# xxxupeng/stereo_toolbox

Hardware: AMD Instinct MI355X
Metric: stereo pairs/sec @ 540x960 D=192 (GwcNet_GC fwd+bwd) (higher is better)
Workload: dtype f32; 1 GPU; GwcNet_GC(maxdisp=192) train step: fwd+bwd+allreduce+Adam, 576x960 pairs (reference pad_to_2x shape), batch 1/GPU, fp32, synthetic randn inputs, deterministic filler weights; global_batch=1, parallelism=dp1, grad_sync=none (single rank: flat fp32 buffer packed, no collective), launch=eager, optimizer=torch.optim.Adam(fused=True)

## Files before the change

### include/stx_hip.h

```cpp
#ifndef STX_HIP_H
#define STX_HIP_H
#ifdef __cplusplus
extern "C" {
#endif

const char* stx_last_error(void);
const char* stx_build_info(void);
int stx_get_tuning(const char* name);
int stx_set_tuning(const char* name, int value);

int stx_cost_volume_fwd(const float* Lg, const float* Rg, int Cg, int G, const float* Lc, const float* Rc, int Cc,
                        const float* scale, float* vol, int B, int H, int W, int D, int mask_left, void* stream);
int stx_group_normalize_fwd(const float* x, float* y, int B, int C, int G, int HW, float out_scale, void* stream);
int stx_group_normalize_bwd(const float* x, const float* gy, float* gx, int B, int C, int G, int HW, float out_scale, void* stream);
int stx_cost_volume_bwd(const float* gvol, const float* Lg, const float* Rg, int Cg, int G, int Cc, float* gLg,
                        float* gRg, float* gLc, float* gRc, int B, int H, int W, int D, int mask_left, void* stream);

int stx_head_fwd(const float* cost, float* disp, float* stats, int B, int Dc, int Hc, int Wc, int D, int H, int W,
                 void* stream);
long long stx_head_bwd_workspace_floats(int B, int Dc, int H, int W);
int stx_head_bwd(const float* gdisp, const float* cost, const float* disp, const float* stats, float* gcost,
                 float* workspace, int B, int Dc, int Hc, int Wc, int D, int H, int W, void* stream);
int stx_head_fwd2(const float* cost, float* disp, float* stats, int B, int Dc, int Hc, int Wc, int D, int H, int W,
                  int align_corners, void* stream);
// ... 9 lines not shown
int stx_softmax_d_fwd(const float* x, float* y, int B, int D, int HW, void* stream);

long long stx_conv3d_packed_floats(int K, int N, int T);
int stx_conv3d_pack_weight(const float* w, float* wp, int A, int B, int T, int mode, void* stream);
int stx_conv3d_fwd_blocks(int Do, int Ho, int Wo);
long long stx_conv3d_fwd_stat_rows(int B, int Di, int Hi, int Wi, int Cin, int Cout, int ks, int stride);
int stx_conv3d_fwd(const float* x, const float* wp, float* out, const float* scale, const float* bias,
                   const float* residual, float* stats, int B, int Di, int Hi, int Wi, int Cin, int Cout, int ks,
                   int stride, int relu, void* stream);
int stx_deconv3d_fwd_blocks(int Di, int Hi, int Wi);
int stx_deconv3d_fwd(const float* x, const float* wp, float* out, const float* scale, const float* bias,
                     const float* residual, float* stats, int B, int Di, int Hi, int Wi, int Cin, int Cout, int Do,
                     int Ho, int Wo, int relu, void* stream);
long long stx_conv3d_wgrad_workspace_floats(int B, int Dc, int Hc, int Wc, int CF, int CC, int ks, int stride);
int stx_conv3d_wgrad(const float* fine, const float* coarse, float* dw, float* workspace, int B, int Df, int Hf, int Wf,
                     int CF, int Dc, int Hc, int Wc, int CC, int ks, int stride, void* stream);

int stx_conv3d_wgrad_bn_supported(int B, int D, int H, int W, int CF, int CC);
int stx_conv3d_wgrad_bn(const float* x, const float* gy, const float* z, const float* scale, const float* shift, const float* mean,
                        const float* invstd, const float* gamma, const float* sums, float inv_n, int act, float* dz, float* dw,
                        float* workspace, int B, int D, int H, int W, int CF, int CC, void* stream);

int stx_conv2d_supported(int Cin, int Cout);
long long stx_conv2d_stat_rows(int groups);
int stx_conv2d_fwd(const float* x, const float* w, float* out, float* stats, int B, int H, int W, int Cin, int Cout, int dgrad,
                   int groups, void* stream);

int stx_conv3d_c1_fwd(const float* x, const float* w, const float* residual, float* out, int B, int D, int H, int W,
                      int Cin, void* stream);
long long stx_conv3d_c1_wgrad_workspace_floats(int Cin);
int stx_conv3d_c1_wgrad(const float* x, const float* gy, float* dw, float* workspace, int B, int D, int H, int W,
                        int Cin, void* stream);
int stx_conv3d_c1_dgrad(const float* gy, const float* w, float* gx, int B, int D, int H, int W, int Cin, void* stream);

int stx_mish_fwd(const float* x, float* y, long long n, void* stream);
int stx_mish_bwd(const float* gy, const float* x, float* gx, long long n, void* stream);
int stx_depth_to_space(const float* y, float* out, int B, int D, int H, int W, int C, int inverse, void* stream);
int stx_gate_fwd(const float* cv, const float* att, float* out, int B, int D, long long HW, int C, void* stream);
int stx_gate_bwd(const float* g, const float* cv, const float* att, float* gcv, float* gatt, int B, int D, long long HW,
                 int C, void* stream);

int stx_concat_channels(const float* in0, const float* in1, const float* in2, const float* in3, int C0, int C1, int C2, int C3,
                        float* out, long long nvox, void* stream);
int stx_split_channels(const float* in, float* out0, float* out1, float* out2, float* out3, int C0, int C1, int C2, int C3,
                       long long nvox, void* stream);
int stx_transpose(const float* in, float* out, int N, int rows, int cols, void* stream);

int stx_dwconv_hw_fwd(const float* x, const float* w, const int* dil, float* out, int B, int D, int H, int W, int C,
                      int flip, void* stream);
long long stx_dwconv_hw_wgrad_workspace_floats(int C);
int stx_dwconv_hw_wgrad(const float* x, const float* gy, const int* dil, float* dw, float* workspace, int B, int D,
                        int H, int W, int C, void* stream);
int stx_cost_volume_scale_bwd(const float* gvol, const float* Lc, const float* Rc, float* gscale, int B, int Cc, int H,
                              int W, int D, int mask_left, void* stream);
int stx_scale_channels(const float* x, const float* s, float* out, long long nvox, int C, void* stream);
int stx_ac_volume_bwd(const float* gvol, const float* Lc, const float* Rc, const float* prob, float* gL, float* gR,
                      float* gprob, int B, int Cc, int H, int W, int D, int mask_left, void* stream);

int stx_bn_reduce_blocks(void);
int stx_bn_stats_rows(long long nvox, int C);
int stx_bn_stats(const float* z, float* partials, long long nvox, int C, int groups, void* stream);
int stx_bn_finalize(const float* partials, int nrows, int C, double count, const float* gamma, const float* beta,
                    float* running_mean, float* running_var, float momentum, float eps, float* scale, float* shift,
                    float* mean, float* invstd, void* stream);
int stx_bn_finalize_groups(const float* partials, int nrows, int C, double count, const float* gamma, const float* beta,
                           float* running_mean, float* running_var, float momentum, float eps, float* out, int groups,
// ... 102 lines not shown
```

### stereo_toolbox_amd/_capi.py

```python
import ctypes
import os
import threading

import torch

_P = ctypes.c_void_p
_I = ctypes.c_int
_F = ctypes.c_float
_L = ctypes.c_longlong

SIGNATURES = {
    "stx_get_tuning": [ctypes.c_char_p],
    "stx_set_tuning": [ctypes.c_char_p, _I],
    "stx_cost_volume_fwd": [_P, _P, _I, _I, _P, _P, _I, _P, _P, _I, _I, _I, _I, _I, _P],
    "stx_cost_volume_bwd": [_P, _P, _P, _I, _I, _I, _P, _P, _P, _P, _I, _I, _I, _I, _I, _P],
    "stx_group_normalize_fwd": [_P, _P, _I, _I, _I, _I, _F, _P],
    "stx_group_normalize_bwd": [_P, _P, _P, _I, _I, _I, _I, _F, _P],
    "stx_head_fwd": [_P, _P, _P, _I, _I, _I, _I, _I, _I, _I, _P],
    "stx_head_bwd_workspace_floats": [_I, _I, _I, _I],
    "stx_head_bwd": [_P, _P, _P, _P, _P, _P, _I, _I, _I, _I, _I, _I, _I, _P],
    "stx_head_fwd2": [_P, _P, _P, _I, _I, _I, _I, _I, _I, _I, _I, _P],
    "stx_head_bwd2": [_P, _P, _P, _P, _P, _P, _I, _I, _I, _I, _I, _I, _I, _I, _P],
    "stx_softargmax_fwd": [_P, _P, _I, _I, _I, _P],
    "stx_argmax_fwd": [_P, _P, _I, _I, _I, _P],
    "stx_softmax_d_fwd": [_P, _P, _I, _I, _I, _P],
    "stx_unimodal_fwd": [_P, _P, _I, _I, _I, _P],
    "stx_dominant_modal_fwd": [_P, _P, _I, _I, _I, _P],
    "stx_modal_fwd": [_P, _P, _P, _I, _I, _I, _I, _P],
    "stx_modal_bwd": [_P, _P, _P, _P, _I, _I, _I, _P],
    "stx_split_mode": [_P, _P, _P, _I, _I, _I, _P],
    "stx_conv3d_packed_floats": [_I, _I, _I],
    "stx_conv3d_pack_weight": [_P, _P, _I, _I, _I, _I, _P],
    "stx_conv3d_fwd_blocks": [_I, _I, _I],
    "stx_conv3d_fwd_stat_rows": [_I, _I, _I, _I, _I, _I, _I, _I],
    "stx_deconv3d_fwd_blocks": [_I, _I, _I],
    "stx_conv3d_fwd": [_P, _P, _P, _P, _P, _P, _P, _I, _I, _I, _I, _I, _I, _I, _I, _I, _P],
    "stx_deconv3d_fwd": [_P, _P, _P, _P, _P, _P, _P, _I, _I, _I, _I, _I, _I, _I, _I, _I, _I, _P],
    "stx_conv3d_wgrad_workspace_floats": [_I, _I, _I, _I, _I, _I, _I, _I],
    "stx_conv3d_wgrad": [_P, _P, _P, _P, _I, _I, _I, _I, _I, _I, _I, _I, _I, _I, _I, _P],
    "stx_conv3d_wgrad_bn_supported": [_I, _I, _I, _I, _I, _I],
    "stx_conv3d_wgrad_bn": [_P] * 9 + [_F, _I, _P, _P, _P, _I, _I, _I, _I, _I, _I, _P],
    "stx_conv2d_supported": [_I, _I],
    "stx_conv2d_stat_rows": [_I],
    "stx_conv2d_fwd": [_P, _P, _P, _P, _I, _I, _I, _I, _I, _I, _I, _P],
    "stx_conv3d_c1_fwd": [_P, _P, _P, _P, _I, _I, _I, _I, _I, _P],
    "stx_conv3d_c1_wgrad_workspace_floats": [_I],
    "stx_conv3d_c1_wgrad": [_P, _P, _P, _P, _I, _I, _I, _I, _I, _P],
    "stx_conv3d_c1_dgrad": [_P, _P, _P, _I, _I, _I, _I, _I, _P],
    "stx_mish_fwd": [_P, _P, _L, _P],
    "stx_mish_bwd": [_P, _P, _P, _L, _P],
    "stx_depth_to_space": [_P, _P, _I, _I, _I, _I, _I, _I, _P],
    "stx_gate_fwd": [_P, _P, _P, _I, _I, _L, _I, _P],
    "stx_gate_bwd": [_P, _P, _P, _P, _P, _I, _I, _L, _I, _P],
    "stx_concat_channels": [_P, _P, _P, _P, _I, _I, _I, _I, _P, _L, _P],
    "stx_split_channels": [_P, _P, _P, _P, _P, _I, _I, _I, _I, _L, _P],
    "stx_transpose": [_P, _P, _I, _I, _I, _P],
    "stx_dwconv_hw_fwd": [_P, _P, _P, _P, _I, _I, _I, _I, _I, _I, _P],
    "stx_dwconv_hw_wgrad_workspace_floats": [_I],
    "stx_dwconv_hw_wgrad": [_P, _P, _P, _P, _P, _I, _I, _I, _I, _I, _P],
    "stx_cost_volume_scale_bwd": [_P, _P, _P, _P, _I, _I, _I, _I, _I, _I, _P],
    "stx_scale_channels": [_P, _P, _P, _L, _I, _P],
    "stx_ac_volume_bwd": [_P, _P, _P, _P, _P, _P, _P, _I, _I, _I, _I, _I, _I, _P],
    "stx_pad_normalize_u8": [_P, _P, _I, _I, _I, _I, _I, _I, _P, _P, _P],
    "stx_warp_fwd": [_P, _P, _P, _I, _I, _I, _I, _P],
    "stx_warp_bwd": [_P, _P, _P, _P, _P, _I, _I, _I, _I, _P],
    "stx_corr_volume_fwd": [_P, _P, _P, _I, _I, _I, _I, _I, _I, _P],
    "stx_corr_volume_bwd": [_P, _P, _P, _P, _P, _I, _I, _I, _I, _I, _I, _P],
    "stx_disparity_variance_fwd": [_P, _P, _P, _P, _I, _I, _I, _P],
    "stx_disparity_variance_bwd": [_P, _P, _P, _P, _P, _P, _P, _I, _I, _I, _P],
    "stx_sampled_volume_fwd": [_P, _P, _I, _I, _P, _P, _I, _P, _P, _I, _I, _I, _I, _I, _P],
    "stx_sampled_volume_bwd": [_P, _P, _P, _I, _I, _I, _P, _P, _P, _P, _P, _I, _I, _I, _I, _I, _P],
    "stx_geo_pyramid_floats": [_L, _I, _I, _I],
    "stx_geo_corr_fwd": [_P, _P, _P, _I, _I, _I, _I, _I, _I, _P],
    "stx_geo_corr_bwd": [_P, _P, _P, _P, _P, _I, _I, _I, _I, _I, _I, _P],
    "stx_geo_pyramid_fwd": [_P, _P, _I, _I, _I, _I, _I, _I, _P],
    "stx_geo_pyramid_bwd": [_P, _P, _I, _I, _I, _I, _I, _I, _P],
    "stx_geo_lookup_fwd": [_P, _P, _P, _P, _P, _I, _I, _I, _I, _I, _I, _I, _I, _P],
    "stx_geo_lookup_bwd": [_P, _P, _P, _P, _P, _I, _I, _I, _I, _I, _I, _I, _I, _P],
    "stx_context_upsample_fwd": [_P, _P, _P, _I, _I, _I, _P],
    "stx_context_upsample_bwd": [_P, _P, _P, _P, _P, _I, _I, _I, _P],
    "stx_corr1d_pyramid_floats": [_L, _I, _I],
# ... 101 lines not shown
```

### stereo_toolbox_amd/aggregation.py

```python
import os
import threading

import torch
import torch.nn as nn

from . import ops


def _is_transposed(conv):
    return isinstance(conv, nn.ConvTranspose3d)


def _conv_cfg(conv):
    ks = conv.kernel_size[0]
    stride = conv.stride[0]
    if _is_transposed(conv):
        k3 = ks == 3 and stride == 2 and conv.padding[0] == 1 and conv.output_padding[0] == 1
        k4 = ks == 4 and stride == 2 and conv.padding[0] == 1 and conv.output_padding[0] == 0
        if not (k3 or k4) or len(set(conv.kernel_size)) != 1 or len(set(conv.stride)) != 1:
            raise ops.StxError("only ConvTranspose3d(k=3, s=2, p=1, op=1) and ConvTranspose3d(k=4, s=2, p=1) are on the hot path")
    else:
        if not ((ks == 3 and conv.padding[0] == 1 and stride in (1, 2)) or (ks == 1 and conv.padding[0] == 0 and stride == 1)):
            raise ops.StxError(f"unsupported Conv3d k={ks} s={stride} p={conv.padding}")
    if conv.bias is not None or conv.groups != 1:
# ... 160 lines not shown
        return _infer_conv(x, conv, s1, b1, residual, relu)

    want = bn is not None and bn.training
    z1, part1 = raw if raw is not None else _raw_conv(x, conv, want)
    if bn is None:
        y = z1
        if residual is not None:
            y = y + residual
        if relu == 3:
            return torch.nn.functional.leaky_relu(y, 0.01)
        return torch.relu(y) if relu else y
    count1 = z1.numel() // z1.shape[-1]
    st1 = _bn_state(bn, part1 if want else None, count1)
    if second is not None:
        x2, conv2, bn2 = second
        want2 = bn2.training
        z2, part2 = second_raw if second_raw is not None else _raw_conv(x2, conv2, want2)
        st2 = _bn_state(bn2, part2 if want2 else None, z2.numel() // z2.shape[-1])
        return ops.BnActFn.apply(z1, bn.weight, bn.bias, z2, bn2.weight, bn2.bias, None, relu, st1, st2)
    defer = (residual is None and want and relu in (0, 1, False, True) and not _is_transposed(conv) and _conv_cfg(conv) == (3, 1)
             and conv.weight.shape[0] % 32 == 0 and conv.weight.shape[1] % 32 == 0 and not st1.get("sync")
             and os.environ.get("STX_BN_BWD_IN_WGRAD", "1") != "0")
    if defer:
        ops.bn_defer_reset_if_stale()
    return ops.BnActFn.apply(z1, bn.weight, bn.bias, None, None, None, residual, relu, st1, None, 1, defer)


@ops.fp32_region
def convbn_block(x, seq, relu=False, second=None, residual=None, mish=False, raw=None, second_raw=None):
    sec = None
    if second is not None:
        sec = (second[0], second[1][0], second[1][1])
    return conv_block(x, seq[0], seq[1], relu=relu, second=sec, residual=residual, mish=mish, raw=raw, second_raw=second_raw)
```

### stereo_toolbox_amd/csrc/conv_c1.hip

```cpp
#include "stx_common.h"
#include <stdlib.h>

namespace {

constexpr int C1_THREADS = 256;
constexpr int C1_TD = 2, C1_TH = 4, C1_TW = 32;
constexpr int C1_ED = C1_TD + 2, C1_EH = C1_TH + 2, C1_EW = C1_TW + 2;
constexpr int C1_CK = 16, C1_VS = C1_CK + 4;

struct C1Args {
    const float* x;
    const float* w;
    const float* gy;
    const float* res;
    float* out;
    int B, D, H, W, Cin;
    int nDt, nHt, nWt, ntiles;
};

__device__ __forceinline__ void c1_stage(const C1Args& a, float* tile, int b, int d0, int h0, int w0, int c0, int tid) {
    for (int idx = tid; idx < C1_ED * C1_EH * C1_EW * (C1_CK / 4); idx += C1_THREADS) {
        const int v = idx / (C1_CK / 4), f = idx - v * (C1_CK / 4);
        const int wx = v % C1_EW, hy = (v / C1_EW) % C1_EH, dz = v / (C1_EW * C1_EH);
        const int gd = d0 - 1 + dz, gh = h0 - 1 + hy, gw = w0 - 1 + wx;
// ... 286 lines not shown
            for (int p = 0; p < 16; ++p) {
                float bv = gp[2 * p];
                bv = (i < 27) ? bv : 0.f;
                acc = __builtin_amdgcn_mfma_f32_32x32x2f32(av[p], bv, acc, 0, 0, 0);
            }
        }
    }
#pragma unroll
    for (int r = 0; r < 16; ++r) red[wave][((r & 3) + 8 * (r >> 2) + 4 * half) * 32 + i] = acc[r];
    __syncthreads();
    float* dst = slab + ((size_t)cb * gridDim.x + blockIdx.x) * 1024;
    for (int idx = tid; idx < 1024; idx += C1_THREADS)
        dst[idx] = (red[0][idx] + red[1][idx]) + (red[2][idx] + red[3][idx]);
}

__global__ __launch_bounds__(C1_THREADS) void c1m_reduce_kernel(const float* __restrict__ slab, int nrows,
                                                                float* __restrict__ dw) {
    __shared__ double red[C1_THREADS];
    const int m = blockIdx.x, tid = threadIdx.x;
    const int tap = m % 27, cfull = m / 27, cb = cfull >> 5, c = cfull & 31;
    const float* p = slab + (size_t)cb * nrows * 1024 + c * 32 + tap;
    double s = 0.0;
    for (int r = tid; r < nrows; r += C1_THREADS) s += (double)p[(size_t)r * 1024];
    red[tid] = s;
    __syncthreads();
    for (int k = C1_THREADS / 2; k > 0; k >>= 1) {
        if (tid < k) red[tid] += red[tid + k];
        __syncthreads();
    }
    if (tid == 0) dw[m] = (float)red[0];
}


constexpr int C1F_TH = 8, C1F_TW = 32;
constexpr int C1F_EH = C1F_TH + 2, C1F_EW = C1F_TW + 2, C1F_NV = C1F_EH * C1F_EW;
constexpr int C1F_MT = (C1F_NV + 31) / 32;
constexpr int C1F_WGS = 512;

__global__ __launch_bounds__(C1_THREADS) void conv_c1_fwd_mfma_kernel(const float* __restrict__ x,
                                                                      const float* __restrict__ w,
                                                                      const float* __restrict__ res,
                                                                      float* __restrict__ out, int B, int D, int H, int W,
                                                                      int nHt, int nWt, int ncols) {
    STX_DYN_SMEM(smem);
    float* Ps = reinterpret_cast<float*>(smem);
    const int tid = threadIdx.x, lane = tid & 63, wave = __builtin_amdgcn_readfirstlane(tid >> 6);
    const int i = lane & 31, half = lane >> 5;
    float wreg[16];
#pragma unroll
    for (int s_ = 0; s_ < 16; ++s_) wreg[s_] = (i < 27) ? w[(size_t)(16 * half + s_) * 27 + i] : 0.f;
    const int lh = tid / C1F_TW, lw = tid % C1F_TW;

    constexpr int MTW = (C1F_MT + 3) / 4;
    const long long units = (long long)ncols * D;
    int u = __builtin_amdgcn_readfirstlane((int)(units * blockIdx.x / gridDim.x));
    const int u_end = __builtin_amdgcn_readfirstlane((int)(units * (blockIdx.x + 1) / gridDim.x));
    const unsigned plane_bytes = (unsigned)H * (unsigned)W * 32u * 4u;
    while (u < u_end) {
        const int col = u / D;
        const int d_lo = u - col * D;
        const int left = u_end - u;
        const int d_hi = (D - d_lo < left) ? D : d_lo + left;
        u += d_hi - d_lo;
        const int wt = col % nWt, ht = (col / nWt) % nHt, b = col / (nWt * nHt);
        const int h0 = ht * C1F_TH, w0 = wt * C1F_TW;
        const int oh = h0 + lh, ow = w0 + lw;
        const bool ook = oh < H && ow < W;
        unsigned voff[MTW];
#pragma unroll
        for (int t = 0; t < MTW; ++t) {
            const int hv = (wave + 4 * t) * 32 + i;
            const int hy = hv / C1F_EW, wx = hv - hy * C1F_EW;
            const int gh = h0 - 1 + hy, gw = w0 - 1 + wx;
            const bool ok = wave + 4 * t < C1F_MT && hv < C1F_NV && gh >= 0 && gh < H && gw >= 0 && gw < W;
            voff[t] = ok ? (unsigned)(((gh * W + gw) * 32 + 16 * half) * 4) : STX_BUF_OOB;
        }
        float4 nxt[MTW][4];
        auto load_plane = [&](int p) {
            const bool in = p >= 0 && p < D && p <= d_hi;
            const stx_bufrsrc rs = stx_make_rsrc(x + ((size_t)b * D + (in ? p : 0)) * H * W * 32, in ? plane_bytes : 0u);
#pragma unroll
            for (int t = 0; t < MTW; ++t)
#pragma unroll
                for (int q = 0; q < 4; ++q) nxt[t][q] = stx_buf_ld4(rs, voff[t], 16u * q);
        };
        float accA = 0.f, accB = 0.f;
        load_plane(d_lo - 1);
        __syncthreads();
        for (int p = d_lo - 1; p <= d_hi; ++p) {
            float* Pb = Ps + ((p + 2) & 1) * (C1F_NV * 27);
            const bool pin = p >= 0 && p < D;
            float4 cur[MTW][4];
#pragma unroll
            for (int t = 0; t < MTW; ++t)
#pragma unroll
                for (int q = 0; q < 4; ++q) cur[t][q] = nxt[t][q];
            load_plane(p + 1);
            if (pin) {
#pragma unroll
                for (int t = 0; t < MTW; ++t) {
                    const int m = wave + 4 * t;
                    if (m < C1F_MT) {
                        f32x16 acc;
#pragma unroll
                        for (int r = 0; r < 16; ++r) acc[r] = 0.f;
#pragma unroll
                        for (int q = 0; q < 4; ++q) {
                            acc = __builtin_amdgcn_mfma_f32_32x32x2f32(cur[t][q].x, wreg[4 * q + 0], acc, 0, 0, 0);
                            acc = __builtin_amdgcn_mfma_f32_32x32x2f32(cur[t][q].y, wreg[4 * q + 1], acc, 0, 0, 0);
                            acc = __builtin_amdgcn_mfma_f32_32x32x2f32(cur[t][q].z, wreg[4 * q + 2], acc, 0, 0, 0);
                            acc = __builtin_amdgcn_mfma_f32_32x32x2f32(cur[t][q].w, wreg[4 * q + 3], acc, 0, 0, 0);
                        }
                        if (i < 27) {
#pragma unroll
                            for (int r = 0; r < 16; ++r) {
                                const int v = m * 32 + (r & 3) + 8 * (r >> 2) + 4 * half;
                                if (v < C1F_NV) Pb[v * 27 + i] = acc[r];
                            }
                        }
                    }
                }
            }
            __syncthreads();
            float s0 = 0.f, s1 = 0.f, s2 = 0.f;
            if (pin) {
#pragma unroll
                for (int kh = 0; kh < 3; ++kh)
#pragma unroll
                    for (int kw = 0; kw < 3; ++kw) {
                        const float* pp = Pb + ((lh + kh) * C1F_EW + lw + kw) * 27 + kh * 3 + kw;
                        s0 += pp[0];
                        s1 += pp[9];
                        s2 += pp[18];
                    }
            }
            const float done = accA + s2;
            const int od = p - 1;
            if (od >= d_lo && od < d_hi && ook) {
                const size_t o = (((size_t)b * D + od) * H + oh) * W + ow;
                out[o] = res ? done + res[o] : done;
            }
            accA = accB + s1;
            accB = s0;
        }
    }
}

}

extern "C" int stx_conv3d_c1_fwd(const float* x, const float* w, const float* residual, float* out, int B, int D,
                                 int H, int W, int Cin, void* stream) {
    stx_begin();
    STX_REQUIRE(x && w && out && B > 0 && D > 0 && H > 0 && W > 0, "conv3d_c1_fwd: bad shape");
    STX_REQUIRE(Cin % C1_CK == 0, "conv3d_c1_fwd: Cin=%d must be a multiple of %d", Cin, C1_CK);
    if (Cin == 32 && (long long)H * W * 128 < (1ll << 31)) {
        const int nHt = stx_cdiv(H, C1F_TH), nWt = stx_cdiv(W, C1F_TW);
        const long long ncols = (long long)B * nHt * nWt, units = ncols * D;
        STX_REQUIRE(units < (1ll << 31), "conv3d_c1_fwd: volume too large");
        long long g = C1F_WGS;
        if (g > units / 4) g = units / 4 > 0 ? units / 4 : 1;
        const size_t lds = (size_t)2 * C1F_NV * 27 * 4;
        if (int rc = stx_lds_require((const void*)conv_c1_fwd_mfma_kernel, lds, "conv3d_c1_fwd(mfma)")) return rc;
        hipLaunchKernelGGL(conv_c1_fwd_mfma_kernel, dim3((unsigned)g), dim3(C1_THREADS), lds, (hipStream_t)stream, x, w,
                           residual, out, B, D, H, W, nHt, nWt, (int)ncols);
        return stx_check_launch("conv3d_c1_fwd(mfma)");
    }
    C1Args a;
    a.x = x; a.w = w; a.gy = nullptr; a.res = residual; a.out = out;
    a.B = B; a.D = D; a.H = H; a.W = W; a.Cin = Cin;
    a.nDt = stx_cdiv(D, C1_TD); a.nHt = stx_cdiv(H, C1_TH); a.nWt = stx_cdiv(W, C1_TW);
    a.ntiles = B * a.nDt * a.nHt * a.nWt;
    if (int rc = stx_lds_require((const void*)conv_c1_fwd_kernel, C1_TILE_BYTES, "conv3d_c1_fwd")) return rc;
    hipLaunchKernelGGL(conv_c1_fwd_kernel, dim3(a.ntiles), dim3(C1_THREADS), C1_TILE_BYTES, (hipStream_t)stream, a);
    return stx_check_launch("conv3d_c1_fwd");
}

extern "C" long long stx_conv3d_c1_wgrad_workspace_floats(int Cin) {
    const long long valu = (long long)C1_WGRAD_BLOCKS * Cin * 27;
    const long long mfma = (long long)C1M_BLOCKS * 1024 * ((Cin + 31) / 32);
    return valu > mfma ? valu : mfma;
}

extern "C" int stx_conv3d_c1_wgrad(const float* x, const float* gy, float* dw, float* workspace, int B, int D, int H,
                                   int W, int Cin, void* stream) {
    stx_begin();
    STX_REQUIRE(x && gy && dw && workspace && B > 0, "conv3d_c1_wgrad: null operand");
    STX_REQUIRE(Cin % C1_CK == 0 && Cin <= 4 * C1_CK, "conv3d_c1_wgrad: Cin=%d must be 16..64 in steps of 16", Cin);
    if (Cin % 32 == 0) {
        const int nDt = stx_cdiv(D, C1M_TD), nHt = stx_cdiv(H, C1M_TH), nWt = stx_cdiv(W, C1M_TW);
        const long long nt = (long long)B * nDt * nHt * nWt;
        STX_REQUIRE(nt < (1ll << 31), "conv3d_c1_wgrad: volume too large");
        const int nblk = nt < C1M_BLOCKS ? (int)nt : C1M_BLOCKS;
        hipStream_t st = (hipStream_t)stream;
        hipLaunchKernelGGL(conv_c1_wgrad_mfma_kernel, dim3(nblk, Cin / 32), dim3(C1_THREADS), 0, st, x, gy, workspace, B,
                           D, H, W, Cin, nDt, nHt, nWt, (int)nt);
        int rc = stx_check_launch("conv3d_c1_wgrad(mfma)");
        if (rc) return rc;
        hipLaunchKernelGGL(c1m_reduce_kernel, dim3(Cin * 27), dim3(C1_THREADS), 0, st, workspace, nblk, dw);
        return stx_check_launch("conv3d_c1_wgrad(reduce)");
    }
    C1Args a;
    a.x = x; a.w = nullptr; a.gy = gy; a.res = nullptr; a.out = workspace;
    a.B = B; a.D = D; a.H = H; a.W = W; a.Cin = Cin;
    a.nDt = stx_cdiv(D, C1_TD); a.nHt = stx_cdiv(H, C1_TH); a.nWt = stx_cdiv(W, C1_TW);
    a.ntiles = B * a.nDt * a.nHt * a.nWt;
    const int nblk = a.ntiles < C1_WGRAD_BLOCKS ? a.ntiles : C1_WGRAD_BLOCKS;
    const size_t lds = C1_TILE_BYTES + 256 * 4;
// ... 26 lines not shown
```

### stereo_toolbox_amd/models/GwcNet/gwcnet.py

```python
import torch
import torch.nn as nn

from ... import ops
from ...aggregation import conv_block, convbn_block, deferred_bn_counters, shared_input_convs
from ..features2d import ResTrunk, cat_features, channels_last_weights_, convbn, init_reference_style, run_head2d, run_pair
from .submodule import convbn_3d


class feature_extraction(ResTrunk):
    fused_everywhere = True

    def __init__(self, concat_feature=False, concat_feature_channel=12):
        super().__init__()
        self.concat_feature = concat_feature
        if concat_feature:
            self.lastconv = nn.Sequential(convbn(320, 128, 3, 1, 1, 1), nn.ReLU(inplace=True),
                                          nn.Conv2d(128, concat_feature_channel, 1, bias=False))

    def forward(self, x):
        gwc = cat_features(self.trunk(x))
        if not self.concat_feature:
            return {"gwc_feature": gwc}
        return {"gwc_feature": gwc, "concat_feature": run_head2d(self.lastconv, gwc)}


class hourglass(nn.Module):

    def __init__(self, c):
        super().__init__()
        self.conv1 = nn.Sequential(convbn_3d(c, c * 2, 3, 2, 1), nn.ReLU(inplace=True))
        self.conv2 = nn.Sequential(convbn_3d(c * 2, c * 2, 3, 1, 1), nn.ReLU(inplace=True))
        self.conv3 = nn.Sequential(convbn_3d(c * 2, c * 4, 3, 2, 1), nn.ReLU(inplace=True))
        self.conv4 = nn.Sequential(convbn_3d(c * 4, c * 4, 3, 1, 1), nn.ReLU(inplace=True))
        self.conv5 = nn.Sequential(nn.ConvTranspose3d(c * 4, c * 2, 3, padding=1, output_padding=1, stride=2, bias=False),
                                   nn.BatchNorm3d(c * 2))
        self.conv6 = nn.Sequential(nn.ConvTranspose3d(c * 2, c, 3, padding=1, output_padding=1, stride=2, bias=False),
                                   nn.BatchNorm3d(c))
        self.redir1 = convbn_3d(c, c, kernel_size=1, stride=1, pad=0)
        self.redir2 = convbn_3d(c * 2, c * 2, kernel_size=1, stride=1, pad=0)

    def forward(self, x, mid=None, also=None):
        rx = shared_input_convs(x, [self.conv1[0], self.redir1] + ([also] if also is not None else []))
        rx = rx or [None, None, None]
        c1 = convbn_block(x, self.conv1[0], relu=True, raw=rx[0])
        c2 = convbn_block(c1, self.conv2[0], relu=True)
        r2 = shared_input_convs(c2, [self.conv3[0], self.redir2]) or [None, None]
        c3 = convbn_block(c2, self.conv3[0], relu=True, raw=r2[0])
        c4 = convbn_block(c3, self.conv4[0], relu=True)
        if mid is not None:
            c4 = mid(c4)
        c5 = convbn_block(c4, self.conv5, relu=True, second=(c2, self.redir2), second_raw=r2[1])
        out = convbn_block(c5, self.conv6, relu=True, second=(x, self.redir1), second_raw=rx[1])
        return (out, rx[2]) if also is not None else out


def classifier(c):
    return nn.Sequential(convbn_3d(c, c, 3, 1, 1), nn.ReLU(inplace=True),
                         nn.Conv3d(c, 1, kernel_size=3, padding=1, stride=1, bias=False))


def run_classifier(seq, x, add=None, raw=None):
    h = convbn_block(x, seq[0], relu=True, raw=raw)
    cost = conv_block(h, seq[2], residual=None if add is None else add.unsqueeze(-1))
    return cost.squeeze(-1)


class GwcNet(nn.Module):
    def __init__(self, maxdisp, use_concat_volume=False):
        super().__init__()
        self.maxdisp = maxdisp
        self.use_concat_volume = use_concat_volume
        self.num_groups = 40
        if use_concat_volume:
            self.concat_channels = 12
            self.feature_extraction = feature_extraction(True, self.concat_channels)
        else:
            self.concat_channels = 0
            self.feature_extraction = feature_extraction(False)
        self.dres0 = nn.Sequential(convbn_3d(self.num_groups + self.concat_channels * 2, 32, 3, 1, 1),
                                   nn.ReLU(inplace=True), convbn_3d(32, 32, 3, 1, 1), nn.ReLU(inplace=True))
        self.dres1 = nn.Sequential(convbn_3d(32, 32, 3, 1, 1), nn.ReLU(inplace=True), convbn_3d(32, 32, 3, 1, 1))
        self.dres2 = hourglass(32)
        self.dres3 = hourglass(32)
        self.dres4 = hourglass(32)
        self.classif0 = classifier(32)
        self.classif1 = classifier(32)
        self.classif2 = classifier(32)
        self.classif3 = classifier(32)
        init_reference_style(self)
        channels_last_weights_(self.feature_extraction)

    def forward(self, left, right):
        with deferred_bn_counters():
            fl, fr = run_pair(self.feature_extraction, left, right, self.training)
            return self.aggregate(fl, fr, left.shape[2], left.shape[3])

# ... 28 lines not shown
```

### stereo_toolbox_amd/models/PSMNet/stackhourglass.py

```python
import torch.nn as nn

from ... import ops
from ...aggregation import conv_block, convbn_block, deferred_bn_counters
from ..features2d import channels_last_weights_, init_reference_style, run_pair
from .submodule import convbn_3d, feature_extraction


class hourglass(nn.Module):

    def __init__(self, inplanes):
        super().__init__()
        c = inplanes
        self.conv1 = nn.Sequential(convbn_3d(c, c * 2, kernel_size=3, stride=2, pad=1), nn.ReLU(inplace=True))
        self.conv2 = convbn_3d(c * 2, c * 2, kernel_size=3, stride=1, pad=1)
        self.conv3 = nn.Sequential(convbn_3d(c * 2, c * 2, kernel_size=3, stride=2, pad=1), nn.ReLU(inplace=True))
        self.conv4 = nn.Sequential(convbn_3d(c * 2, c * 2, kernel_size=3, stride=1, pad=1), nn.ReLU(inplace=True))
        self.conv5 = nn.Sequential(nn.ConvTranspose3d(c * 2, c * 2, kernel_size=3, padding=1, output_padding=1,
                                                      stride=2, bias=False), nn.BatchNorm3d(c * 2))
        self.conv6 = nn.Sequential(nn.ConvTranspose3d(c * 2, c, kernel_size=3, padding=1, output_padding=1,
                                                      stride=2, bias=False), nn.BatchNorm3d(c))

    def forward(self, x, presqu, postsqu, skip=None):
        out = convbn_block(x, self.conv1[0], relu=True)
        pre = convbn_block(out, self.conv2, relu=True, residual=postsqu)
        out = convbn_block(pre, self.conv3[0], relu=True)
        out = convbn_block(out, self.conv4[0], relu=True)
        post = convbn_block(out, self.conv5, relu=True, residual=presqu if presqu is not None else pre)
        out = convbn_block(post, self.conv6, relu=False, residual=skip)
        return out, pre, post


def _classifier():
    return nn.Sequential(convbn_3d(32, 32, 3, 1, 1), nn.ReLU(inplace=True),
                         nn.Conv3d(32, 1, kernel_size=3, padding=1, stride=1, bias=False))


def _run_classifier(seq, x, add=None):
    h = convbn_block(x, seq[0], relu=True)
    cost = conv_block(h, seq[2], residual=None if add is None else add.unsqueeze(-1))
    return cost.squeeze(-1)


class PSMNet(nn.Module):
    def __init__(self, maxdisp=192):
        super().__init__()
        self.maxdisp = maxdisp
        self.feature_extraction = feature_extraction()
        self.dres0 = nn.Sequential(convbn_3d(64, 32, 3, 1, 1), nn.ReLU(inplace=True),
                                   convbn_3d(32, 32, 3, 1, 1), nn.ReLU(inplace=True))
        self.dres1 = nn.Sequential(convbn_3d(32, 32, 3, 1, 1), nn.ReLU(inplace=True), convbn_3d(32, 32, 3, 1, 1))
        self.dres2 = hourglass(32)
        self.dres3 = hourglass(32)
        self.dres4 = hourglass(32)
        self.classif1 = _classifier()
        self.classif2 = _classifier()
        self.classif3 = _classifier()
        init_reference_style(self)
        channels_last_weights_(self.feature_extraction)

    def forward(self, left, right):
        with deferred_bn_counters():
            fl, fr = run_pair(self.feature_extraction, left, right, self.training)
            return self.aggregate(fl, fr, left.shape[2], left.shape[3])

    @ops.fp32_region
    def aggregate(self, fl, fr, H, W):
        cost = ops.cost_volume(None, None, fl, fr, self.maxdisp // 4, 0, mask_left=True)
        cost0 = convbn_block(cost, self.dres0[0], relu=True)
        cost0 = convbn_block(cost0, self.dres0[2], relu=True)
        t = convbn_block(cost0, self.dres1[0], relu=True)
        cost0 = convbn_block(t, self.dres1[2], relu=False, residual=cost0)
        out1, pre1, post1 = self.dres2(cost0, None, None, skip=cost0)
# ... 12 lines not shown
```

### stereo_toolbox_amd/ops.py

```python
import ctypes

import torch

from ._capi import StxError, get_lib

_P = ctypes.c_void_p


class _DevPtr(ctypes.c_void_p):
    """A device pointer that remembers the device of the tensor it came from: _call() reads the launch device off its
    own arguments, so nothing survives between launches (an exception between building the arguments and the launch
    cannot leak state into the next one)."""


def _stream(dev=None):
    return _P(torch.cuda.current_stream(dev).cuda_stream)


def _p(t):
    if t is None:
        return None
    p = _DevPtr(t.data_ptr())
    p.dev = t.device
    return p


def on_device(t):
    return t.is_cuda


def _chk(t, name, dims=None):
    if t is None:
        return
# ... 787 lines not shown
            return (None, tot[1], tot[0], None, None, None, None, None, None, None, None, None)
        if (ctx.defer and not ctx.two and not ctx.has_res and ctx.relu in (0, 1) and ctx.train1 and not ctx.sync and G == 1
                and (not ctx.relu or ctx.remask)):
            alias = gy.view_as(gy)
            pend = _PendingBn()
            pend.g, pend.z, pend.scale, pend.shift, pend.mean, pend.invstd = alias, z1, sc1, sh1, m1, i1
            pend.gamma, pend.sums, pend.inv_n, pend.act = gamma1, sums, 1.0 / nvox, int(ctx.relu)
            if pend.scale is None:
                pend.scale = pend.shift = m1
            _defer_pending_bn(alias, pend)
            tot = sums_all[0]
            return (alias, tot[1], tot[0], None, None, None, None, None, None, None, None, None)
        dz1 = torch.empty_like(z1)
        dz2 = torch.empty_like(z2) if ctx.two else None
        gres = torch.empty_like(z1) if (ctx.has_res and ctx.relu) else None
        use = sums
        if ctx.sync:
            import torch.distributed as dist
            use = sums.clone()
            dist.all_reduce(use, group=ctx.sync[0])
            use /= ctx.sync[1]
        if not ctx.train1 or (ctx.two and not ctx.train2):
            use = torch.zeros_like(sums)
        _call("stx_bn_bwd_apply2", _p(gy), _p(y), _p(z1), _p(m1), _p(i1), _p(gamma1), _p(z2) if ctx.two else None,
              _p(m2) if ctx.two else None, _p(i2) if ctx.two else None, _p(gamma2) if ctx.two else None, _p(sc1), _p(sh1),
              _p(sc2), _p(sh2), _p(use), _p(dz1), _p(dz2), _p(gres), nvox, C, int(ctx.relu), G)
        if ctx.has_res and not ctx.relu:
            gres = gy
        tot = sums_all[G] if G > 1 else sums_all[0]
        return (dz1, tot[1], tot[0], dz2, tot[2] if ctx.two else None, tot[0].clone() if ctx.two else None, gres,
                None, None, None, None, None)


class MishFn(torch.autograd.Function):

    @staticmethod
    def forward(ctx, x):
        x = x.contiguous()
        _chk(x, "x")
        y = torch.empty_like(x)
        _call("stx_mish_fwd", _p(x), _p(y), x.numel())
        ctx.save_for_backward(x)
        return y

    @staticmethod
    def backward(ctx, gy):
        (x,) = ctx.saved_tensors
        gy = gy.contiguous()
        gx = torch.empty_like(x)
        _call("stx_mish_bwd", _p(gy), _p(x), _p(gx), x.numel())
        return gx


@fp32_region
def mish(x):
    if torch.is_grad_enabled() and x.requires_grad:
        return MishFn.apply(x)
    x = x.contiguous()
    _chk(x, "x")
    y = torch.empty_like(x)
    _call("stx_mish_fwd", _p(x), _p(y), x.numel())
    return y


def _cv_shapes(Lg, Lc, num_groups):
    ref = Lg if Lg is not None else Lc
# ... 1114 lines not shown
```

Measured before the change: 0.1788 pairs/s.

## Fuse classifier BN+ReLU into the 32→1 conv3d forward and backward

Adds a classifier_block path where the train-mode BatchNorm apply and ReLU feed straight into the 32-to-1 channel 3x3x3 conv. The forward applies scale, shift and activation on the fly inside the MFMA conv kernel, so the activated tensor is never materialised. The backward computes the input gradient, BN reduction sums and weight gradient in one tiled kernel plus a small reduction kernel, then defers the BN gradient apply. This removes full-volume reads and writes of the 32-channel activation, at the cost of recomputing the activation in backward and extra code restricted to specific shapes.

```diff
diff --git a/include/stx_hip.h b/include/stx_hip.h
--- a/include/stx_hip.h
+++ b/include/stx_hip.h
@@ -65,6 +65,12 @@
 int stx_conv3d_c1_wgrad(const float* x, const float* gy, float* dw, float* workspace, int B, int D, int H, int W,
                         int Cin, void* stream);
 int stx_conv3d_c1_dgrad(const float* gy, const float* w, float* gx, int B, int D, int H, int W, int Cin, void* stream);
+int stx_conv3d_c1_fwd_bn(const float* z, const float* scale, const float* shift, int act, const float* w,
+                         const float* residual, float* out, int B, int D, int H, int W, void* stream);
+long long stx_conv3d_c1_bwd_bn_workspace_floats(void);
+int stx_conv3d_c1_bwd_bn(const float* gcost, const float* w, const float* z, const float* scale, const float* shift,
+                         const float* mean, const float* invstd, int act, float* gh, float* sums, float* dw,
+                         float* workspace, int B, int D, int H, int W, void* stream);
 
 int stx_mish_fwd(const float* x, float* y, long long n, void* stream);
 int stx_mish_bwd(const float* gy, const float* x, float* gx, long long n, void* stream);
diff --git a/stereo_toolbox_amd/_capi.py b/stereo_toolbox_amd/_capi.py
--- a/stereo_toolbox_amd/_capi.py
+++ b/stereo_toolbox_amd/_capi.py
@@ -47,6 +47,9 @@
     "stx_conv3d_c1_wgrad_workspace_floats": [_I],
     "stx_conv3d_c1_wgrad": [_P, _P, _P, _P, _I, _I, _I, _I, _I, _P],
     "stx_conv3d_c1_dgrad": [_P, _P, _P, _I, _I, _I, _I, _I, _P],
+    "stx_conv3d_c1_fwd_bn": [_P, _P, _P, _I, _P, _P, _P, _I, _I, _I, _I, _P],
+    "stx_conv3d_c1_bwd_bn_workspace_floats": [],
+    "stx_conv3d_c1_bwd_bn": [_P] * 7 + [_I, _P, _P, _P, _P, _I, _I, _I, _I, _P],
     "stx_mish_fwd": [_P, _P, _L, _P],
     "stx_mish_bwd": [_P, _P, _P, _L, _P],
     "stx_depth_to_space": [_P, _P, _I, _I, _I, _I, _I, _I, _P],
diff --git a/stereo_toolbox_amd/aggregation.py b/stereo_toolbox_amd/aggregation.py
--- a/stereo_toolbox_amd/aggregation.py
+++ b/stereo_toolbox_amd/aggregation.py
@@ -216,3 +216,22 @@
     if second is not None:
         sec = (second[0], second[1][0], second[1][1])
     return conv_block(x, seq[0], seq[1], relu=relu, second=sec, residual=residual, mish=mish, raw=raw, second_raw=second_raw)
+
+
+@ops.fp32_region
+def classifier_block(x, seq, add=None, raw=None):
+    conv, bn, c1 = seq[0][0], seq[0][1], seq[2]
+    z_grad = raw[0].requires_grad if raw is not None else _needs_grad(x, conv)
+    fused = (ops.c1_fused_enabled() and os.environ.get("STX_BN_BWD_IN_WGRAD", "1") != "0" and torch.is_grad_enabled()
+             and bn.training and not isinstance(bn, nn.SyncBatchNorm) and isinstance(conv, nn.Conv3d)
+             and not _is_transposed(conv) and _conv_cfg(conv) == (3, 1) and tuple(conv.weight.shape[:2]) == (32, 32)
+             and isinstance(c1, nn.Conv3d) and tuple(c1.weight.shape) == (1, 32, 3, 3, 3) and _conv_cfg(c1) == (3, 1)
+             and x.dim() == 5 and x.shape[2] * x.shape[3] * 128 < (1 << 31)
+             and z_grad and bn.weight.requires_grad and c1.weight.requires_grad)
+    if not fused:
+        h = convbn_block(x, seq[0], relu=True, raw=raw)
+        return conv_block(h, c1, residual=add)
+    ops.bn_defer_reset_if_stale()
+    z1, part1 = raw if raw is not None else _raw_conv(x, conv, True)
+    st1 = _bn_state(bn, part1, z1.numel() // z1.shape[-1])
+    return ops.BnActC1Fn.apply(z1, bn.weight, bn.bias, c1.weight, add, st1)
diff --git a/stereo_toolbox_amd/csrc/conv_c1.hip b/stereo_toolbox_amd/csrc/conv_c1.hip
--- a/stereo_toolbox_amd/csrc/conv_c1.hip
+++ b/stereo_toolbox_amd/csrc/conv_c1.hip
@@ -342,16 +342,143 @@
 }
 
 
+constexpr int C1B_BLOCKS = 768;
+
+__global__ __launch_bounds__(C1_THREADS) void conv_c1_bwd_bn_kernel(
+    const float* __restrict__ gy, const float* __restrict__ w, const float* __restrict__ z, const float* __restrict__ scale,
+    const float* __restrict__ shift, const float* __restrict__ mean, const float* __restrict__ invstd, int act,
+    float* __restrict__ gx, float* __restrict__ bnrows, float* __restrict__ slab, int B, int D, int H, int W, int nHt, int nWt,
+    int ntiles) {
+    __shared__ float gys[3 * C1D_EH * C1D_EW];
+    __shared__ float red[4][1024];
+    const int tid = threadIdx.x, lane = tid & 63, wave = tid >> 6;
+    const int i = lane & 31, half = lane >> 5;
+    float wreg[14];
+    int aoff[14];
+#pragma unroll
+    for (int j = 0; j < 14; ++j) {
+        const int tap = 2 * j + half;
+        const int tp = tap < 27 ? tap : 26;
+        const int kd = tp / 9, kh = (tp / 3) % 3, kw = tp % 3;
+        wreg[j] = tap < 27 ? w[(size_t)i * 27 + tap] : 0.f;
+        aoff[j] = ((2 - kd) * C1D_EH + (wave + 2 - kh)) * C1D_EW + i + 2 - kw;
+    }
+    const int bkd = i / 9, bkh = (i / 3) % 3, bkw = i % 3;
+    const int boff = (i < 27) ? ((2 - bkd) * C1D_EH + (wave + 2 - bkh)) * C1D_EW + (2 - bkw) + 4 * half : 0;
+    const float sc = scale[i], sh = shift[i], mu = mean[i], is = invstd[i];
+    float s0 = 0.f, s1 = 0.f;
+    f32x16 wacc;
+#pragma unroll
+    for (int r = 0; r < 16; ++r) wacc[r] = 0.f;
+    const unsigned plane_bytes = (unsigned)H * (unsigned)W * 128u;
+    for (int tile = blockIdx.x; tile < ntiles; tile += gridDim.x) {
+        int r_ = tile;
+        const int wt = r_ % nWt; r_ /= nWt;
+        const int ht = r_ % nHt; r_ /= nHt;
+        const int d = r_ % D;
+        const int b = r_ / D;
+        const int h0 = ht * C1D_TH, w0 = wt * C1D_TW;
+        const int oh = h0 + wave;
+        const size_t plane = ((size_t)b * D + d) * H * W * 32;
+        const stx_bufrsrc ors = stx_make_rsrc(gx + plane, plane_bytes);
+        const stx_bufrsrc zrs = stx_make_rsrc(z + plane, plane_bytes);
+        const unsigned vbase = (unsigned)((((oh < H ? oh : 0) * W + w0 + 4 * half) * 32 + i) * 4);
+        float zv[16];
+#pragma unroll
+        for (int r = 0; r < 16; ++r) {
+            const int m = (r & 3) + 8 * (r >> 2);
+            const bool ok = oh < H && w0 + 4 * half + m < W;
+            zv[r] = stx_buf_ld1(zrs, ok ? vbase : STX_BUF_OOB, (unsigned)(m * 128));
+        }
+        __syncthreads();
+        for (int idx = tid; idx < 3 * C1D_EH * C1D_EW; idx += C1_THREADS) {
+            const int wx = idx % C1D_EW, hy = (idx / C1D_EW) % C1D_EH, dz = idx / (C1D_EW * C1D_EH);
+            const int gd = d - 1 + dz, gh = h0 - 1 + hy, gw = w0 - 1 + wx;
+            gys[idx] = (gd >= 0 && gd < D && gh >= 0 && gh < H && gw >= 0 && gw < W)
+                           ? gy[(((size_t)b * D + gd) * H + gh) * W + gw] : 0.f;
+        }
+        __syncthreads();
+        f32x16 acc;
+#pragma unroll
+        for (int r = 0; r < 16; ++r) acc[r] = 0.f;
+        float av[14];
+#pragma unroll
+        for (int j = 0; j < 14; ++j) av[j] = gys[aoff[j]];
+#pragma unroll
+        for (int j = 0; j < 14; ++j) acc = __builtin_amdgcn_mfma_f32_32x32x2f32(av[j], wreg[j], acc, 0, 0, 0);
+        float hv[16];
+#pragma unroll
+        for (int r = 0; r < 16; ++r) {
+            const int m = (r & 3) + 8 * (r >> 2);
+            const bool ok = oh < H && w0 + 4 * half + m < W;
+            stx_buf_st1(ors, ok ? vbase : STX_BUF_OOB, (unsigned)(m * 128), acc[r]);
+            const float pre = fmaf(zv[r], sc, sh);
+            const float g = ok ? (act ? stx_act_bwd(acc[r], pre, act) : acc[r]) : 0.f;
+            s0 += g;
+            s1 = fmaf(g, (zv[r] - mu) * is, s1);
+            hv[r] = ok ? stx_act(pre, act) : 0.f;
+        }
+#pragma unroll
+        for (int r = 0; r < 16; ++r) {
+            float bv = gys[boff + (r & 3) + 8 * (r >> 2)];
+            bv = (i < 27) ? bv : 0.f;
+            wacc = __builtin_amdgcn_mfma_f32_32x32x2f32(hv[r], bv, wacc, 0, 0, 0);
+        }
+    }
+    red[0][tid] = s0;
+    red[1][tid] = s1;
+    __syncthreads();
+    if (tid < 64) {
+        const float* p = red[tid >> 5] + (tid & 31);
+        bnrows[(size_t)blockIdx.x * 64 + tid] =
+            ((p[0] + p[32]) + (p[64] + p[96])) + ((p[128] + p[160]) + (p[192] + p[224]));
+    }
+    __syncthreads();
+#pragma unroll
+    for (int r = 0; r < 16; ++r) red[wave][((r & 3) + 8 * (r >> 2) + 4 * half) * 32 + i] = wacc[r];
+    __syncthreads();
+    float* dst = slab + (size_t)blockIdx.x * 1024;
+    for (int idx = tid; idx < 1024; idx += C1_THREADS)
+        dst[idx] = (red[0][idx] + red[1][idx]) + (red[2][idx] + red[3][idx]);
+}
+
+__global__ __launch_bounds__(C1_THREADS) void c1b_reduce_kernel(const float* __restrict__ slab,
+                                                                const float* __restrict__ bnrows, int nrows,
+                                                                float* __restrict__ dw, float* __restrict__ sums) {
+    __shared__ double red[C1_THREADS];
+    const int m = blockIdx.x, tid = threadIdx.x;
+    const int q = m - 32 * 27;
+    if (q >= 64) {
+        if (tid == 0) sums[q] = 0.f;
+        return;
+    }
+    const float* p = q >= 0 ? bnrows + q : slab + (m / 27) * 32 + m % 27;
+    const size_t stride = q >= 0 ? 64 : 1024;
+    double s = 0.0;
+    for (int r = tid; r < nrows; r += C1_THREADS) s += (double)p[(size_t)r * stride];
+    red[tid] = s;
+    __syncthreads();
+    for (int k = C1_THREADS / 2; k > 0; k >>= 1) {
+        if (tid < k) red[tid] += red[tid + k];
+        __syncthreads();
+    }
+    if (tid == 0) (q >= 0 ? sums[q] : dw[m]) = (float)red[0];
+}
+
+
 constexpr int C1F_TH = 8, C1F_TW = 32;
 constexpr int C1F_EH = C1F_TH + 2, C1F_EW = C1F_TW + 2, C1F_NV = C1F_EH * C1F_EW;
 constexpr int C1F_MT = (C1F_NV + 31) / 32;
 constexpr int C1F_WGS = 512;
 
+template <bool BN>
 __global__ __launch_bounds__(C1_THREADS) void conv_c1_fwd_mfma_kernel(const float* __restrict__ x,
                                                                       const float* __restrict__ w,
                                                                       const float* __restrict__ res,
-                                                                      float* __restrict__ out, int B, int D, int H, int W,
-                                                                      int nHt, int nWt, int ncols) {
+                                                                      float* __restrict__ out,
+                                                                      const float* __restrict__ scale,
+                                                                      const float* __restrict__ shift, int act, int B, int D,
+                                                                      int H, int W, int nHt, int nWt, int ncols) {
     STX_DYN_SMEM(smem);
     float* Ps = reinterpret_cast<float*>(smem);
     const int tid = threadIdx.x, lane = tid & 63, wave = __builtin_amdgcn_readfirstlane(tid >> 6);
@@ -360,6 +487,12 @@
 #pragma unroll
     for (int s_ = 0; s_ < 16; ++s_) wreg[s_] = (i < 27) ? w[(size_t)(16 * half + s_) * 27 + i] : 0.f;
     const int lh = tid / C1F_TW, lw = tid % C1F_TW;
+    float bsc[16], bsh[16];
+#pragma unroll
+    for (int s_ = 0; s_ < 16; ++s_) {
+        bsc[s_] = BN ? scale[16 * half + s_] : 1.f;
+        bsh[s_] = BN ? shift[16 * half + s_] : 0.f;
+    }
 
     constexpr int MTW = (C1F_MT + 3) / 4;
     const long long units = (long long)ncols * D;
@@ -414,6 +547,17 @@
                         f32x16 acc;
 #pragma unroll
                         for (int r = 0; r < 16; ++r) acc[r] = 0.f;
+                        if (BN) {
+                            const bool vok = voff[t] != STX_BUF_OOB;
+#pragma unroll
+                            for (int q = 0; q < 4; ++q) {
+                                float4& a = cur[t][q];
+                                a.x = vok ? stx_act(fmaf(a.x, bsc[4 * q + 0], bsh[4 * q + 0]), act) : 0.f;
+                                a.y = vok ? stx_act(fmaf(a.y, bsc[4 * q + 1], bsh[4 * q + 1]), act) : 0.f;
+                                a.z = vok ? stx_act(fmaf(a.z, bsc[4 * q + 2], bsh[4 * q + 2]), act) : 0.f;
+                                a.w = vok ? stx_act(fmaf(a.w, bsc[4 * q + 3], bsh[4 * q + 3]), act) : 0.f;
+                            }
+                        }
 #pragma unroll
                         for (int q = 0; q < 4; ++q) {
                             acc = __builtin_amdgcn_mfma_f32_32x32x2f32(cur[t][q].x, wreg[4 * q + 0], acc, 0, 0, 0);
@@ -458,23 +602,33 @@
 
 }
 
+static int c1_fwd_mfma_launch(const float* x, const float* w, const float* residual, float* out, const float* scale,
+                              const float* shift, int act, int B, int D, int H, int W, void* stream) {
+    const int nHt = stx_cdiv(H, C1F_TH), nWt = stx_cdiv(W, C1F_TW);
+    const long long ncols = (long long)B * nHt * nWt, units = ncols * D;
+    STX_REQUIRE(units < (1ll << 31), "conv3d_c1_fwd: volume too large");
+    long long g = C1F_WGS;
+    if (g > units / 4) g = units / 4 > 0 ? units / 4 : 1;
+    const size_t lds = (size_t)2 * C1F_NV * 27 * 4;
+    if (scale) {
+        if (int rc = stx_lds_require((const void*)conv_c1_fwd_mfma_kernel<true>, lds, "conv3d_c1_fwd_bn(mfma)")) return rc;
+        hipLaunchKernelGGL(conv_c1_fwd_mfma_kernel<true>, dim3((unsigned)g), dim3(C1_THREADS), lds, (hipStream_t)stream, x, w,
+                           residual, out, scale, shift, act, B, D, H, W, nHt, nWt, (int)ncols);
+        return stx_check_launch("conv3d_c1_fwd_bn(mfma)");
+    }
+    if (int rc = stx_lds_require((const void*)conv_c1_fwd_mfma_kernel<false>, lds, "conv3d_c1_fwd(mfma)")) return rc;
+    hipLaunchKernelGGL(conv_c1_fwd_mfma_kernel<false>, dim3((unsigned)g), dim3(C1_THREADS), lds, (hipStream_t)stream, x, w,
+                       residual, out, scale, shift, act, B, D, H, W, nHt, nWt, (int)ncols);
+    return stx_check_launch("conv3d_c1_fwd(mfma)");
+}
+
 extern "C" int stx_conv3d_c1_fwd(const float* x, const float* w, const float* residual, float* out, int B, int D,
                                  int H, int W, int Cin, void* stream) {
     stx_begin();
     STX_REQUIRE(x && w && out && B > 0 && D > 0 && H > 0 && W > 0, "conv3d_c1_fwd: bad shape");
     STX_REQUIRE(Cin % C1_CK == 0, "conv3d_c1_fwd: Cin=%d must be a multiple of %d", Cin, C1_CK);
-    if (Cin == 32 && (long long)H * W * 128 < (1ll << 31)) {
-        const int nHt = stx_cdiv(H, C1F_TH), nWt = stx_cdiv(W, C1F_TW);
-        const long long ncols = (long long)B * nHt * nWt, units = ncols * D;
-        STX_REQUIRE(units < (1ll << 31), "conv3d_c1_fwd: volume too large");
-        long long g = C1F_WGS;
-        if (g > units / 4) g = units / 4 > 0 ? units / 4 : 1;
-        const size_t lds = (size_t)2 * C1F_NV * 27 * 4;
-        if (int rc = stx_lds_require((const void*)conv_c1_fwd_mfma_kernel, lds, "conv3d_c1_fwd(mfma)")) return rc;
-        hipLaunchKernelGGL(conv_c1_fwd_mfma_kernel, dim3((unsigned)g), dim3(C1_THREADS), lds, (hipStream_t)stream, x, w,
-                           residual, out, B, D, H, W, nHt, nWt, (int)ncols);
-        return stx_check_launch("conv3d_c1_fwd(mfma)");
-    }
+    if (Cin == 32 && (long long)H * W * 128 < (1ll << 31))
+        return c1_fwd_mfma_launch(x, w, residual, out, nullptr, nullptr, 0, B, D, H, W, stream);
     C1Args a;
     a.x = x; a.w = w; a.gy = nullptr; a.res = residual; a.out = out;
     a.B = B; a.D = D; a.H = H; a.W = W; a.Cin = Cin;
@@ -483,6 +637,39 @@
     if (int rc = stx_lds_require((const void*)conv_c1_fwd_kernel, C1_TILE_BYTES, "conv3d_c1_fwd")) return rc;
     hipLaunchKernelGGL(conv_c1_fwd_kernel, dim3(a.ntiles), dim3(C1_THREADS), C1_TILE_BYTES, (hipStream_t)stream, a);
     return stx_check_launch("conv3d_c1_fwd");
+}
+
+extern "C" int stx_conv3d_c1_fwd_bn(const float* z, const float* scale, const float* shift, int act, const float* w,
+                                    const float* residual, float* out, int B, int D, int H, int W, void* stream) {
+    stx_begin();
+    STX_REQUIRE(z && scale && shift && w && out && B > 0 && D > 0 && H > 0 && W > 0, "conv3d_c1_fwd_bn: bad shape");
+    STX_REQUIRE(act >= 0 && act <= 3, "conv3d_c1_fwd_bn: activation code %d", act);
+    STX_REQUIRE((long long)H * W * 128 < (1ll << 31), "conv3d_c1_fwd_bn: plane %d x %d beyond the descriptor range", H, W);
+    return c1_fwd_mfma_launch(z, w, residual, out, scale, shift, act, B, D, H, W, stream);
+}
+
+extern "C" long long stx_conv3d_c1_bwd_bn_workspace_floats(void) { return (long long)C1B_BLOCKS * (1024 + 64); }
+
+extern "C" int stx_conv3d_c1_bwd_bn(const float* gcost, const float* w, const float* z, const float* scale,
+                                    const float* shift, const float* mean, const float* invstd, int act, float* gh,
+                                    float* sums, float* dw, float* workspace, int B, int D, int H, int W, void* stream) {
+    stx_begin();
+    STX_REQUIRE(gcost && w && z && scale && shift && mean && invstd && gh && sums && dw && workspace,
+                "conv3d_c1_bwd_bn: null operand");
+    STX_REQUIRE(B > 0 && D > 0 && H > 0 && W > 0, "conv3d_c1_bwd_bn: bad shape");
+    STX_REQUIRE(act >= 0 && act <= 3, "conv3d_c1_bwd_bn: activation code %d", act);
+    STX_REQUIRE((long long)H * W * 128 < (1ll << 31), "conv3d_c1_bwd_bn: plane %d x %d beyond the descriptor range", H, W);
+    const int nHt = stx_cdiv(H, C1D_TH), nWt = stx_cdiv(W, C1D_TW);
+    const long long nt = (long long)B * D * nHt * nWt;
+    STX_REQUIRE(nt < (1ll << 31), "conv3d_c1_bwd_bn: volume too large");
+    const int nblk = nt < C1B_BLOCKS ? (int)nt : C1B_BLOCKS;
+    float* bnrows = workspace + (size_t)C1B_BLOCKS * 1024;
+    hipStream_t st = (hipStream_t)stream;
+    hipLaunchKernelGGL(conv_c1_bwd_bn_kernel, dim3(nblk), dim3(C1_THREADS), 0, st, gcost, w, z, scale, shift, mean, invstd, act,
+                       gh, bnrows, workspace, B, D, H, W, nHt, nWt, (int)nt);
+    if (int rc = stx_check_launch("conv3d_c1_bwd_bn")) return rc;
+    hipLaunchKernelGGL(c1b_reduce_kernel, dim3(32 * 27 + 96), dim3(C1_THREADS), 0, st, workspace, bnrows, nblk, dw, sums);
+    return stx_check_launch("conv3d_c1_bwd_bn(reduce)");
 }
 
 extern "C" long long stx_conv3d_c1_wgrad_workspace_floats(int Cin) {
diff --git a/stereo_toolbox_amd/models/GwcNet/gwcnet.py b/stereo_toolbox_amd/models/GwcNet/gwcnet.py
--- a/stereo_toolbox_amd/models/GwcNet/gwcnet.py
+++ b/stereo_toolbox_amd/models/GwcNet/gwcnet.py
@@ -2,7 +2,7 @@
 import torch.nn as nn
 
 from ... import ops
-from ...aggregation import conv_block, convbn_block, deferred_bn_counters, shared_input_convs
+from ...aggregation import classifier_block, convbn_block, deferred_bn_counters, shared_input_convs
 from ..features2d import ResTrunk, cat_features, channels_last_weights_, convbn, init_reference_style, run_head2d, run_pair
 from .submodule import convbn_3d
 
@@ -60,8 +60,7 @@
 
 
 def run_classifier(seq, x, add=None, raw=None):
-    h = convbn_block(x, seq[0], relu=True, raw=raw)
-    cost = conv_block(h, seq[2], residual=None if add is None else add.unsqueeze(-1))
+    cost = classifier_block(x, seq, add=None if add is None else add.unsqueeze(-1), raw=raw)
     return cost.squeeze(-1)
 
 
diff --git a/stereo_toolbox_amd/models/PSMNet/stackhourglass.py b/stereo_toolbox_amd/models/PSMNet/stackhourglass.py
--- a/stereo_toolbox_amd/models/PSMNet/stackhourglass.py
+++ b/stereo_toolbox_amd/models/PSMNet/stackhourglass.py
@@ -1,7 +1,7 @@
 import torch.nn as nn
 
 from ... import ops
-from ...aggregation import conv_block, convbn_block, deferred_bn_counters
+from ...aggregation import classifier_block, convbn_block, deferred_bn_counters
 from ..features2d import channels_last_weights_, init_reference_style, run_pair
 from .submodule import convbn_3d, feature_extraction
 
@@ -36,8 +36,7 @@
 
 
 def _run_classifier(seq, x, add=None):
-    h = convbn_block(x, seq[0], relu=True)
-    cost = conv_block(h, seq[2], residual=None if add is None else add.unsqueeze(-1))
+    cost = classifier_block(x, seq, add=None if add is None else add.unsqueeze(-1))
     return cost.squeeze(-1)
 
 
diff --git a/stereo_toolbox_amd/ops.py b/stereo_toolbox_amd/ops.py
--- a/stereo_toolbox_amd/ops.py
+++ b/stereo_toolbox_amd/ops.py
@@ -1,4 +1,5 @@
 import ctypes
+import os
 
 import torch
 
@@ -852,6 +853,46 @@
                 None, None, None, None, None)
 
 
+def c1_fused_enabled():
+    return os.environ.get("STX_C1_FUSED", "1") != "0"
+
+
+class BnActC1Fn(torch.autograd.Function):
+
+    @staticmethod
+    def forward(ctx, z1, gamma, beta, w_c1, add, bn):
+        _chk(z1, "z1", 5)
+        _chk(add, "add", 5)
+        B, D, H, W, C = z1.shape
+        if C != 32 or tuple(w_c1.shape) != (1, 32, 3, 3, 3) or not bn["training"] or bn.get("sync"):
+            raise StxError("BnActC1Fn: a 32-channel head behind a train-mode plain BatchNorm only")
+        sc, sh, m, i = bn_finalize(bn["partials"], bn["count"], gamma, beta, bn["running_mean"], bn["running_var"],
+                                   bn["momentum"], bn["eps"])
+        w = w_c1.contiguous()
+        cost = torch.empty(B, D, H, W, 1, dtype=torch.float32, device=z1.device)
+        _call("stx_conv3d_c1_fwd_bn", _p(z1), _p(sc), _p(sh), 1, _p(w), _p(add), _p(cost), B, D, H, W)
+        ctx.save_for_backward(z1, sc, sh, m, i, gamma, w)
+        return cost
+
+    @staticmethod
+    def backward(ctx, gcost):
+        z1, sc, sh, m, i, gamma, w = ctx.saved_tensors
+        gcost = gcost.contiguous()
+        B, D, H, W, C = z1.shape
+        ws = _WS.get("c1bwdbn", get_lib().raw("stx_conv3d_c1_bwd_bn_workspace_floats")(), z1.device)
+        gh = torch.empty_like(z1)
+        sums = torch.empty(1, 3, C, dtype=torch.float32, device=z1.device)
+        dw = torch.empty(1, C, 3, 3, 3, dtype=torch.float32, device=z1.device)
+        _call("stx_conv3d_c1_bwd_bn", _p(gcost), _p(w), _p(z1), _p(sc), _p(sh), _p(m), _p(i), 1, _p(gh), _p(sums), _p(dw),
+              _p(ws), B, D, H, W)
+        alias = gh.view_as(gh)
+        pend = _PendingBn()
+        pend.g, pend.z, pend.scale, pend.shift, pend.mean, pend.invstd = alias, z1, sc, sh, m, i
+        pend.gamma, pend.sums, pend.inv_n, pend.act = gamma, sums, 1.0 / (z1.numel() // C), 1
+        _defer_pending_bn(alias, pend)
+        return alias, sums[0, 1], sums[0, 0], dw, (gcost if ctx.needs_input_grad[4] else None), None
+
+
 class MishFn(torch.autograd.Function):
 
     @staticmethod
```

After: 0.1787 pairs/s. No clear change (-0.1%).
